# Z-yq/TensorflowASR

Measured on AMD Instinct MI355X. Metric: audio-frames/sec/GPU + RTF, ConformerCTC(S) 10s utts, 1/2/4/8 MI355X, higher is better.
Workload: dtype f32

## Files before the change

### tensorflowasr_amd/csrc/attention_split.hip

```cpp
#include <cstdlib>

#include "common.h"
#include "env.h"
#include "launch.h"
#include "mfma_ops.h"

MI355_SCALAR_F32_BEGIN

namespace {

#ifndef MI355ASR_ATTN_DIAG
#define MI355ASR_ATTN_DIAG 0
#endif
constexpr int ADG = MI355ASR_ATTN_DIAG;
constexpr int HS = 36;
constexpr int TPK = 256;
constexpr int NKT = TPK / 16;
constexpr int NST = TPK / 32;
constexpr int OT = 3;
constexpr int AW = 16;
constexpr int ATH = AW * 64;

template <int TM>
__global__ __launch_bounds__(ATH) void attention_split_kernel(AttnArgs a) {
  static_assert(TM == 3 || ADG == 0, "the timing variants are those of the three-term kernel");
  __shared__ __attribute__((aligned(16))) u32x4_t Kf[TM][NKT][64];
  __shared__ __attribute__((aligned(16))) float Kt[NKT][64];
  __shared__ __attribute__((aligned(16))) u32x4_t Vf[TM][NST][OT][64];
  const float sq = TM == 2 ? a.h2_sq : 1.f, sk = TM == 2 ? a.h2_sk : 1.f, sv = TM == 2 ? a.h2_sv : 1.f;
  constexpr float SP = TM == 2 ? 16384.f : 1.f;

  const int tid = threadIdx.x, lane = tid & 63, wv = tid >> 6;
  const int g = lane >> 4, g4 = g * 4, c = lane & 15;
  const int TS = a.Tk, TQ = a.Tq;
  const int h = blockIdx.y, b = blockIdx.z;
  const int T = a.k_len ? min(a.k_len[b], TS) : TS;
  const int ld = a.ldk, D = a.D;
  const size_t khead = a.head_major ? ((size_t)b * a.H + h) * TS * HS : (size_t)b * TS * ld + h * HS;
  const float* __restrict__ kbase = a.k + khead;
  const float* __restrict__ vbase = a.v + khead;

  const int qt = blockIdx.x * AW + wv;
  const int tq = qt * 16 + c;
  const float* qrow = a.head_major ? a.q + (((size_t)b * a.H + h) * TQ + min(tq, TQ - 1)) * HS
                                   : a.q + ((size_t)b * TQ + min(tq, TQ - 1)) * a.ldq + h * HS;
  constexpr float LOG2E = 1.4426950408889634f;
  const f32x4 qlo = ldg4(qrow + 8 * g), qhi = ldg4(qrow + 8 * g + 4);
  const float qtl = qrow[32 + g] * (LOG2E * sq);

  const int skey = 16 * wv + c;
  const float* krow = kbase + (size_t)min(skey, T - 1) * ld;
  f32x4 klo = ldg4(krow + 8 * g), khi = ldg4(krow + 8 * g + 4);
  float ktl = krow[32 + g];
  constexpr int NVE = NST * OT * 64, NVT = (NVE + ATH - 1) / ATH;
  float ve[NVT][8];
#pragma unroll
  for (int it = 0; it < NVT; ++it) {
    const int en = tid + it * ATH;
    const int s = en / (OT * 64), rem = en - s * (OT * 64), ot = rem >> 6, l = rem & 63, kg = l >> 4, fc = l & 15;
    const int f = 16 * ot + fc;
#pragma unroll
    for (int j = 0; j < 8; ++j) {
      const int key = 32 * s + 16 * (j >> 2) + 4 * kg + (j & 3);
      ve[it][j] = (!(ADG & 16) && en < NVE && f < HS && key < T) ? vbase[(size_t)key * ld + f] : 0.f;
    }
  }
  if (skey >= T) { klo = splat4(0.f); khi = splat4(0.f); ktl = 0.f; }
  {
    const Split8x3 kf = split_tm<TM>(klo * splat4(sk), khi * splat4(sk));
    Kf[0][wv][lane] = kf.t[0];
    Kf[1][wv][lane] = kf.t[1];
    if constexpr (TM == 3) Kf[2][wv][lane] = kf.t[2];
    Kt[wv][lane] = ktl * sk;
  }
  __syncthreads();
  const bool active = qt * 16 < TQ;
  const int nkt = (T + 15) / 16;
  const Split8x3 qf = split_tm<TM>(qlo * splat4(LOG2E * sq), qhi * splat4(LOG2E * sq));
  const f32x4 inv_qk = splat4(1.0f / (sq * sk));

  f32x4 sc[NKT];
  auto qk_tile = [&](int kt) {
    const u32x4_t kf[3] = {Kf[0][kt][lane], Kf[1][kt][lane], Kf[TM - 1][kt][lane]};
    const float kl = Kt[kt][lane];
    if constexpr (ADG & 1) { sc[kt] = splat4(kl) + __builtin_bit_cast(f32x4, kf[0]); return; }
    f32x4 acc = mma_tm<TM>(kf, qf, splat4(0.f));
    sc[kt] = mfma4(kl, qtl, acc);
    if constexpr (TM == 2) sc[kt] = sc[kt] * inv_qk;
  };
  const bool full = (nkt == NKT);
  if (active) {
    if (full) {
#pragma unroll
      for (int kt = 0; kt < NKT; ++kt) qk_tile(kt);
    } else {
#pragma unroll
      for (int kt = 0; kt < NKT; ++kt) {
        if (kt < nkt) qk_tile(kt); else sc[kt] = splat4(-INFINITY);
      }
    }
  }

#pragma unroll
  for (int it = 0; it < NVT; ++it) {
    const int en = tid + it * ATH;
    if (en < NVE && !(ADG & 8)) {
      const f32x4 lo = {ve[it][0], ve[it][1], ve[it][2], ve[it][3]}, hi = {ve[it][4], ve[it][5], ve[it][6], ve[it][7]};
      const Split8x3 vf = split_tm<TM>(lo * splat4(sv), hi * splat4(sv));
      u32x4_t* dst = &Vf[0][0][0][0] + en;
      dst[0] = vf.t[0];
      dst[NVE] = vf.t[1];
      if constexpr (TM == 3) dst[2 * NVE] = vf.t[2];
    }
  }
  if (!active) { __syncthreads(); return; }

  float mx = -INFINITY;
#pragma unroll
  for (int kt = 0; kt < NKT; ++kt) {
    if (kt < nkt && 16 * kt + 16 > T) {
      const int kb = 16 * kt + g4;
      sc[kt].x = (kb + 0 < T) ? sc[kt].x : -INFINITY;
      sc[kt].y = (kb + 1 < T) ? sc[kt].y : -INFINITY;
      sc[kt].z = (kb + 2 < T) ? sc[kt].z : -INFINITY;
      sc[kt].w = (kb + 3 < T) ? sc[kt].w : -INFINITY;
    }
    mx = fmaxf(mx, fmaxf(fmaxf(sc[kt].x, sc[kt].y), fmaxf(sc[kt].z, sc[kt].w)));
  }
  mx = group_max(mx);
  float psum = 0.f;
#pragma unroll
  for (int kt = 0; kt < NKT; ++kt) {
    if constexpr (!(ADG & 2)) {
      sc[kt].x = __builtin_amdgcn_exp2f(sc[kt].x - mx);
      sc[kt].y = __builtin_amdgcn_exp2f(sc[kt].y - mx);
      sc[kt].z = __builtin_amdgcn_exp2f(sc[kt].z - mx);
      sc[kt].w = __builtin_amdgcn_exp2f(sc[kt].w - mx);
    }
    psum += (sc[kt].x + sc[kt].y) + (sc[kt].z + sc[kt].w);
  }

  __syncthreads();
  f32x4 o[OT];
#pragma unroll
  for (int i = 0; i < OT; ++i) o[i] = splat4(0.f);
  const int nst = (nkt + 1) / 2;
#pragma unroll
  for (int s = 0; s < NST; ++s) {
    if constexpr (ADG & 4) { o[0] += sc[2 * s]; o[1] += sc[2 * s + 1]; }
    else if (s < nst) {
      const Split8x3 pf = split_tm<TM>(sc[2 * s] * splat4(SP), sc[2 * s + 1] * splat4(SP));
#pragma unroll
      for (int i = 0; i < OT; ++i) {
        const u32x4_t vf[3] = {Vf[0][s][i][lane], Vf[1][s][i][lane], Vf[TM - 1][s][i][lane]};
        o[i] = mma_tm<TM>(vf, pf, o[i]);
      }
    }
  }
  const float inv = (1.0f / group_sum(psum)) * (1.0f / (SP * sv));
  if (tq < TQ) {
    float* orow = a.ctx + ((size_t)b * TQ + tq) * D + h * HS;
#pragma unroll
    for (int i = 0; i < OT; ++i) {
      if (16 * i + g4 < HS) stg4(orow + 16 * i + g4, o[i] * splat4(inv));
    }
  }
}


constexpr int LKB = 256;
constexpr int LKT = LKB / 16;
constexpr int LST = LKB / 32;
template <int TM, int LW>
__global__ __launch_bounds__(LW * 64) void attention_split_long_kernel(AttnArgs a) {
  constexpr int LTH = LW * 64;
  constexpr bool LPRE = LW <= 8;
  __shared__ __attribute__((aligned(16))) u32x4_t Kf[TM][LKT][64];
  __shared__ __attribute__((aligned(16))) float Kt[LKT][64];
  __shared__ __attribute__((aligned(16))) u32x4_t Vf[TM][LST][OT][64];
  const float sq = TM == 2 ? a.h2_sq : 1.f, sk = TM == 2 ? a.h2_sk : 1.f, sv = TM == 2 ? a.h2_sv : 1.f;
  constexpr float SP = TM == 2 ? 16384.f : 1.f;
  const int tid = threadIdx.x, lane = tid & 63, wv = tid >> 6;
  const int g = lane >> 4, g4 = g * 4, c = lane & 15;
  const int TS = a.Tk, TQ = a.Tq;
  const int h = blockIdx.y, b = blockIdx.z;
  const int T = a.k_len ? min(a.k_len[b], TS) : TS;
  const int ld = a.ldk, D = a.D;
  const size_t khead = a.head_major ? ((size_t)b * a.H + h) * TS * HS : (size_t)b * TS * ld + h * HS;
  const float* __restrict__ kbase = a.k + khead;
  const float* __restrict__ vbase = a.v + khead;
  const int qt = blockIdx.x * LW + wv;
  const int tq = qt * 16 + c;
  const float* qrow = a.head_major ? a.q + (((size_t)b * a.H + h) * TQ + min(tq, TQ - 1)) * HS
                                   : a.q + ((size_t)b * TQ + min(tq, TQ - 1)) * a.ldq + h * HS;
  constexpr float LOG2E = 1.4426950408889634f;
  const f32x4 qlo = ldg4(qrow + 8 * g), qhi = ldg4(qrow + 8 * g + 4);
  const float qtl = qrow[32 + g] * (LOG2E * sq);
  const Split8x3 qf = split_tm<TM>(qlo * splat4(LOG2E * sq), qhi * splat4(LOG2E * sq));
  const f32x4 inv_qk = splat4(1.0f / (sq * sk));
  const bool active = qt * 16 < TQ;

  constexpr int NKE = LKT * 64, NKR = (NKE + LTH - 1) / LTH;
  constexpr int NVE = LST * OT * 64, NVR = (NVE + LTH - 1) / LTH;
  f32x4 klo[NKR], khi[NKR];
  float ktl[NKR];
  float ve[NVR][8];
  const unsigned uld = (unsigned)ld;
  auto fetch = [&](int kb0) {
#pragma unroll
    for (int it = 0; it < NKR; ++it) {
      const int en = tid + it * LTH, kt = en >> 6, l = en & 63, kg = l >> 4, kc = l & 15;
      const int skey = kb0 + 16 * kt + kc;
      const unsigned ko = (unsigned)min(skey, T - 1) * uld + 8u * kg;
      const bool ok = en < NKE && skey < T;
      klo[it] = ok ? *reinterpret_cast<const f32x4*>(kbase + ko) : splat4(0.f);
      khi[it] = ok ? *reinterpret_cast<const f32x4*>(kbase + ko + 4u) : splat4(0.f);
      ktl[it] = ok ? kbase[(unsigned)min(skey, T - 1) * uld + 32u + kg] : 0.f;
    }
#pragma unroll
    for (int it = 0; it < NVR; ++it) {
      const int en = tid + it * LTH;
      const int s = en / (OT * 64), rem = en - s * (OT * 64), ot = rem >> 6, l = rem & 63, kg = l >> 4, fc = l & 15;
      const int f = 16 * ot + fc;
      const int key0 = kb0 + 32 * s + 4 * kg;
      const unsigned vo = (unsigned)key0 * uld + (unsigned)f;
#pragma unroll
      for (int j = 0; j < 8; ++j) {
        const int dk = 16 * (j >> 2) + (j & 3);
        ve[it][j] = (en < NVE && f < HS && key0 + dk < T) ? vbase[vo + (unsigned)dk * uld] : 0.f;
      }
    }
  };
  auto stage = [&]() {
#pragma unroll
    for (int it = 0; it < NKR; ++it) {
      const int en = tid + it * LTH;
      if (en < NKE) {
        const Split8x3 kf = split_tm<TM>(klo[it] * splat4(sk), khi[it] * splat4(sk));
        (&Kf[0][0][0])[en] = kf.t[0];
        (&Kf[1][0][0])[en] = kf.t[1];
        if constexpr (TM == 3) (&Kf[2][0][0])[en] = kf.t[2];
        (&Kt[0][0])[en] = ktl[it] * sk;
      }
    }
#pragma unroll
    for (int it = 0; it < NVR; ++it) {
      const int en = tid + it * LTH;
      if (en < NVE) {
        const f32x4 lo = {ve[it][0], ve[it][1], ve[it][2], ve[it][3]}, hi = {ve[it][4], ve[it][5], ve[it][6], ve[it][7]};
        const Split8x3 vf = split_tm<TM>(lo * splat4(sv), hi * splat4(sv));
        u32x4_t* dst = &Vf[0][0][0][0] + en;
        dst[0] = vf.t[0];
        dst[NVE] = vf.t[1];
        if constexpr (TM == 3) dst[2 * NVE] = vf.t[2];
      }
    }
  };

  float m = -INFINITY, psum = 0.f;
  f32x4 o[OT];
#pragma unroll
  for (int i = 0; i < OT; ++i) o[i] = splat4(0.f);
  if constexpr (LPRE) fetch(0);
#pragma unroll 1
  for (int kb0 = 0; kb0 < T; kb0 += LKB) {
    if constexpr (!LPRE) fetch(kb0);
    stage();
// ... 119 lines not shown
```

### tensorflowasr_amd/csrc/subconv.hip

```cpp
#include <cstdio>
#include <cstdlib>

#include "common.h"
#include "env.h"
#include "launch.h"
#include "wstream.h"
#include "mfma_ops.h"

MI355_SCALAR_F32_BEGIN

namespace {

constexpr int D = 144;
constexpr int KB = D / 16;
constexpr int NB = KB;

struct SubCtx {
  float win[7][7];
  unsigned valid;
  int g4;
  const float *p_w1, *p_b1;
};

struct SubState {
  f32x4 xf;
  f32x4 tw[2][2];
};

DEV f32x4 rd_tap(const float* w1c, int tp) {
  int off = tp * D;
  asm volatile("" : "+v"(off));
  return *reinterpret_cast<const f32x4*>(w1c + off);
}
DEV void tap(f32x4& v, const SubCtx& cx, int q, int tp, const f32x4 w) {
  const int kt = q / 3, kf = q % 3, i = tp / 3, j = tp % 3;
  float m = cx.win[2 * kt + i][2 * kf + j];
  asm volatile("" : "+v"(m));
  v.x = __builtin_fmaf(m, w.x, v.x); v.y = __builtin_fmaf(m, w.y, v.y);
  v.z = __builtin_fmaf(m, w.z, v.z); v.w = __builtin_fmaf(m, w.w, v.w);
}
DEV f32x4 finish(f32x4 v, const SubCtx& cx, int q) {
  const bool ok = (cx.valid >> q) & 1u;
  v.x = ok ? fmaxf(v.x, 0.f) : 0.f; v.y = ok ? fmaxf(v.y, 0.f) : 0.f;
  v.z = ok ? fmaxf(v.z, 0.f) : 0.f; v.w = ok ? fmaxf(v.w, 0.f) : 0.f;
  return v;
}

template <int CUR0>
DEV void channel_block(f32x4 (&acc)[NB], WStream<NB>& ws, SubState& st, unsigned l16, const SubCtx& cx, int cb,
                       const f32x4* __restrict__ w2) {
  const int cbn = min(cb + 1, KB - 1);
  const float* w1c = cx.p_w1 + 16 * cb + cx.g4;
  const float* w1n = cx.p_w1 + 16 * cbn + cx.g4;
  const f32x4 b1v = lds4(cx.p_b1, cb, cx.g4), b1n = lds4(cx.p_b1, cbn, cx.g4);
  static_for<0, 9>([&](auto Q) {
    constexpr int q = decltype(Q)::value;
    constexpr int qn = (q + 1) % 9;
    const int sidx = cb * 9 + q;
    const f32x4* p1 = w2 + (size_t)min(sidx + 1, 9 * KB - 1) * (KB * 64);
    const f32x4* p2 = w2 + (size_t)min(sidx + 2, 9 * KB - 1) * (KB * 64);
    f32x4 xn = (q < 8) ? b1v : b1n;
    batch_step<(CUR0 + q) & 1>(acc, st.xf, ws, l16, p1, p2, [&](auto GI) {
      constexpr int gi = decltype(GI)::value;
      constexpr int h = CUR0 + q * 5 + gi;
      tap(xn, cx, qn, 2 * gi, st.tw[h & 1][0]);
      if constexpr (gi < 4) tap(xn, cx, qn, 2 * gi + 1, st.tw[h & 1][1]);
      if constexpr (gi == 4) xn = finish(xn, cx, qn);
      constexpr int gn = (gi + 1) % 5;
      const float* wsrc = (q < 7 || (q == 7 && gi < 4)) ? w1c : w1n;
      st.tw[(h + 1) & 1][0] = rd_tap(wsrc, 2 * gn);
      if constexpr (gn < 4) st.tw[(h + 1) & 1][1] = rd_tap(wsrc, 2 * gn + 1);
    });
    st.xf = xn;
  });
}

__global__ __launch_bounds__(BLOCK_THREADS, 2) void subconv144_kernel(SubConvArgs a) {
  __shared__ __attribute__((aligned(16))) float p_w1[9 * D], p_b1[D], p_b2[D];
  const int lane = threadIdx.x & 63;
  const int g4 = (lane >> 4) * 4, c = lane & 15;
  const int wid = blockIdx.x * WAVES_PER_BLOCK + (threadIdx.x >> 6);
  const int P = a.B * a.T2 * a.F2;

  SubCtx cx;
  cx.g4 = g4; cx.p_w1 = p_w1; cx.p_b1 = p_b1;
  const int pos = wid * 16 + c;
  {
    const int p = min(pos, P - 1);
    const int b = p / (a.T2 * a.F2);
    const int r = p % (a.T2 * a.F2);
    const int t2 = r / a.F2, f2 = r % a.F2;
    int F = a.F, T1 = a.T1, pt1 = a.pt1, pt2 = a.pt2;
    if (a.wav_len) {
      int t2_;
      F = (a.wav_len[b] + a.hop - 1) / a.hop;
      ragged_same_pad(F, 3, a.st1, &T1, &pt1);
      ragged_same_pad(T1, 3, 2, &t2_, &pt2);
    }
    const int tm0 = 4 * t2 - 2 * pt2 - pt1;
    const int fm0 = 4 * f2 - 2 * a.pf2 - a.pf1;
    const float* __restrict__ mb = a.mel + (size_t)b * a.F * a.NM;
#pragma unroll
    for (int i = 0; i < 7; ++i) {
      const int tm = tm0 + i;
#pragma unroll
      for (int j = 0; j < 7; ++j) {
        const int fm = fm0 + j;
        cx.win[i][j] = (tm >= 0 && tm < F && fm >= 0 && fm < a.NM) ? mb[(size_t)tm * a.NM + fm] : 0.f;
      }
    }
    cx.valid = 0;
#pragma unroll
    for (int kt = 0; kt < 3; ++kt)
#pragma unroll
      for (int kf = 0; kf < 3; ++kf) {
        const int t1 = 2 * t2 + kt - pt2, f1 = 2 * f2 + kf - a.pf2;
        const unsigned ok = (unsigned)((t1 >= 0) & (t1 < T1) & (f1 >= 0) & (f1 < a.F1));
        cx.valid |= ok << (kt * 3 + kf);
      }
  }
  const f32x4* w2 = reinterpret_cast<const f32x4*>(a.w2p);
  WStream<NB> ws;
  ws.lane16 = (unsigned)lane * 16u;
  stream_begin(ws, w2, w2 + (size_t)KB * 64);
  stash(p_w1, a.w1, 9 * D); stash(p_b1, a.b1, D); stash(p_b2, a.b2, D);
  __syncthreads();
  if ((size_t)wid * 16 >= (size_t)P) return;

  f32x4 acc[NB];
#pragma unroll
  for (int n = 0; n < NB; ++n) acc[n] = lds4(p_b2, n, g4);
  SubState st;
  {
    const float* w1c = p_w1 + g4;
    f32x4 v = lds4(p_b1, 0, g4);
#pragma unroll
    for (int tp = 0; tp < 9; ++tp) tap(v, cx, 0, tp, rd_tap(w1c, tp));
    st.xf = finish(v, cx, 0);
    st.tw[0][0] = rd_tap(w1c, 0);
    st.tw[0][1] = rd_tap(w1c, 1);
  }
#pragma unroll 1
  for (int cb = 0; cb + 1 < KB; cb += 2) {
    const unsigned l16 = fresh_lane16(ws.lane16);
    channel_block<0>(acc, ws, st, l16, cx, cb, w2);
    channel_block<1>(acc, ws, st, l16, cx, cb + 1, w2);
  }
  {
    const unsigned l16 = fresh_lane16(ws.lane16);
    channel_block<0>(acc, ws, st, l16, cx, KB - 1, w2);
  }
  if (pos < P) {
    float* orow = a.out + (size_t)pos * D;
#pragma unroll
    for (int n = 0; n < NB; ++n) {
      f32x4 v = acc[n];
      v.x = fmaxf(v.x, 0.f); v.y = fmaxf(v.y, 0.f); v.z = fmaxf(v.z, 0.f); v.w = fmaxf(v.w, 0.f);
      stg4(orow + 16 * n + g4, v);
    }
  }
}


constexpr int SCW = 8, SCT = SCW * 64, SRT = 2, SPOSG = SCW * 16 * SRT;
constexpr int NPAIR = 4;
constexpr int ninth_steps(int kb) { return (kb + 1) / 2; }
constexpr int MELP = 8192;

#ifndef MI355ASR_SUBCONV_C1I
#define MI355ASR_SUBCONV_C1I 1
#endif
#ifndef MI355ASR_SUBCONV_RING
#define MI355ASR_SUBCONV_RING 4
#endif
constexpr int SRING = MI355ASR_SUBCONV_RING;
static_assert(SRING >= 2 && (SRING & (SRING - 1)) == 0, "ring slots: a power of two");
DEV void wait_vmcnt(int n) {
  switch (n) {
    case 0: __builtin_amdgcn_s_waitcnt(0x0f70); break;
    case 2: __builtin_amdgcn_s_waitcnt(0x0f72); break;
    case 3: __builtin_amdgcn_s_waitcnt(0x0f73); break;
    case 4: __builtin_amdgcn_s_waitcnt(0x0f74); break;
    case 6: __builtin_amdgcn_s_waitcnt(0x0f76); break;
    case 8: __builtin_amdgcn_s_waitcnt(0x0f78); break;
    case 9: __builtin_amdgcn_s_waitcnt(0x0f79); break;
    case 12: __builtin_amdgcn_s_waitcnt(0x0f7c); break;
    default: __builtin_amdgcn_s_waitcnt(0x0f70); break;
  }
}

#ifndef MI355ASR_CONV1_V2
#define MI355ASR_CONV1_V2 1
#endif
#define MI355ASR_CONV1_PK MI355ASR_CONV1_V2

template <int RTN, bool PK_ = true>
struct SplitLane {
  static constexpr bool PK = PK_;
  int mb[RTN];
  unsigned valid[RTN];
};

struct PatchGeom { int row, seg; };
#if MI355ASR_CONV1_V2
struct Win9 { float m[3][3]; };
template <int Q, int DIAG = 0, class SL>
DEV Win9 conv1_window(const float* melp, PatchGeom RS, const SL& sl, int rt) {
  constexpr int kt = Q / 3, kf = Q % 3;
  int off = sl.mb[rt];
  asm volatile("" : "+v"(off));
  const float* mp = melp + off + (2 * kt) * RS.row;
  Win9 w;
#pragma unroll
  for (int i = 0; i < 3; ++i) {
    const float* rp = mp + i * RS.row;
    if constexpr (DIAG == 5) {
#pragma unroll
      for (int j = 0; j < 3; ++j) w.m[i][j] = __builtin_bit_cast(float, off + i * RS.row + 2 * kf + j);
    } else if constexpr (kf == 1) {
      const f32x2 a = *reinterpret_cast<const f32x2*>(rp + 2);
      w.m[i][0] = a.x; w.m[i][1] = a.y; w.m[i][2] = rp[4];
    } else {
      const f32x4 a = *reinterpret_cast<const f32x4*>(rp + 2 * kf);
      w.m[i][0] = a.x; w.m[i][1] = a.y; w.m[i][2] = a.z;
    }
  }
  return w;
}
template <int Q, class SL>
DEV f32x4 conv1_eval(const Win9& win, const SL& sl, int rt, const f32x4 (&w1r)[9], f32x4 b1v) {
  f32x2 lo2 = {b1v.x, b1v.y}, hi2 = {b1v.z, b1v.w};
#pragma unroll
  for (int i = 0; i < 3; ++i)
#pragma unroll
    for (int j = 0; j < 3; ++j) {
      const f32x4 w = w1r[i * 3 + j];
      const float m = win.m[i][j];
      if constexpr (SL::PK) {
        const f32x2 mm = {m, m};
        lo2 = __builtin_elementwise_fma(mm, f32x2{w.x, w.y}, lo2);
        hi2 = __builtin_elementwise_fma(mm, f32x2{w.z, w.w}, hi2);
      } else {
        lo2.x = __builtin_fmaf(m, w.x, lo2.x); lo2.y = __builtin_fmaf(m, w.y, lo2.y);
        hi2.x = __builtin_fmaf(m, w.z, hi2.x); hi2.y = __builtin_fmaf(m, w.w, hi2.y);
      }
    }
  const bool ok = (sl.valid[rt] >> Q) & 1u;
  const float lim = ok ? __builtin_inff() : 0.f;
  return f32x4{__builtin_amdgcn_fmed3f(lo2.x, 0.f, lim), __builtin_amdgcn_fmed3f(lo2.y, 0.f, lim),
               __builtin_amdgcn_fmed3f(hi2.x, 0.f, lim), __builtin_amdgcn_fmed3f(hi2.y, 0.f, lim)};
}
template <int Q, int DIAG = 0, class SL>
DEV f32x4 conv1_at(const float* melp, PatchGeom RS, const SL& sl, int rt, const f32x4 (&w1r)[9], f32x4 b1v) {
  return conv1_eval<Q>(conv1_window<Q, DIAG>(melp, RS, sl, rt), sl, rt, w1r, b1v);
}
#else
template <int Q, int DIAG = 0, class SL>
DEV f32x4 conv1_at(const float* melp, PatchGeom RS, const SL& sl, int rt, const f32x4 (&w1r)[9], f32x4 b1v) {
  constexpr int kt = Q / 3, kf = Q % 3;
  f32x4 v = b1v;
  int off = sl.mb[rt];
  asm volatile("" : "+v"(off));
  const float* mp = melp + off + (2 * kt) * RS.row;
#pragma unroll
  for (int i = 0; i < 3; ++i)
#pragma unroll
    for (int j = 0; j < 3; ++j) {
      const int mc = 2 * kf + j, col = (mc & 3) * RS.seg + (mc >> 2);
      const float m = DIAG == 5 ? __builtin_bit_cast(float, off + i * RS.row + col) : mp[i * RS.row + col];
      const f32x4 w = w1r[i * 3 + j];
      v.x = __builtin_fmaf(m, w.x, v.x); v.y = __builtin_fmaf(m, w.y, v.y);
      v.z = __builtin_fmaf(m, w.z, v.z); v.w = __builtin_fmaf(m, w.w, v.w);
    }
  const bool ok = (sl.valid[rt] >> Q) & 1u;
  v.x = ok ? fmaxf(v.x, 0.f) : 0.f; v.y = ok ? fmaxf(v.y, 0.f) : 0.f;
  v.z = ok ? fmaxf(v.z, 0.f) : 0.f; v.w = ok ? fmaxf(v.w, 0.f) : 0.f;
  return v;
}
#endif

template <int PAIR, int DIAG = 0, int TM = 3, int RTN, class SL>
DEV void frags_for(Split8x3 (&xf)[RTN], const float* melp, PatchGeom RS, const SL& sl, const f32x4 (&w1r)[9], f32x4 b1v) {
#pragma unroll
  for (int rt = 0; rt < RTN; ++rt) {
    f32x4 lo, hi;
#if MI355ASR_CONV1_V2
    if constexpr (SL::PK) {
      const Win9 wlo = conv1_window<2 * PAIR, DIAG>(melp, RS, sl, rt), whi = conv1_window<2 * PAIR + 1, DIAG>(melp, RS, sl, rt);
      lo = conv1_eval<2 * PAIR>(wlo, sl, rt, w1r, b1v);
      hi = conv1_eval<2 * PAIR + 1>(whi, sl, rt, w1r, b1v);
    } else
#endif
    {
      lo = conv1_at<2 * PAIR, DIAG>(melp, RS, sl, rt, w1r, b1v);
      hi = conv1_at<2 * PAIR + 1, DIAG>(melp, RS, sl, rt, w1r, b1v);
    }
    if constexpr (DIAG == 6) {
      const u32x4_t l = __builtin_bit_cast(u32x4_t, lo), h = __builtin_bit_cast(u32x4_t, hi);
      xf[rt].t[0] = l; xf[rt].t[1] = h; xf[rt].t[2] = l ^ h;
    } else {
      xf[rt] = split_tm<TM>(lo, hi);
    }
  }
}

template <int DIAG, int TM, class LT, int RTN, class SL>
DEV void frags_ninth(Split8x3 (&xf)[RTN], const float* melp, PatchGeom RS, const SL& sl, f32x4 (&w1r)[9], const float* p_b1,
                     int g4, int cbA, int KBn, LT&& load_taps) {
  f32x4 lo[RTN], hi[RTN];
  load_taps(cbA);
#pragma unroll
  for (int rt = 0; rt < RTN; ++rt) lo[rt] = conv1_at<8, DIAG>(melp, RS, sl, rt, w1r, lds4(p_b1, cbA, g4));
  if (cbA + 1 < KBn) {
    load_taps(cbA + 1);
#pragma unroll
    for (int rt = 0; rt < RTN; ++rt) hi[rt] = conv1_at<8, DIAG>(melp, RS, sl, rt, w1r, lds4(p_b1, cbA + 1, g4));
  } else {
#pragma unroll
    for (int rt = 0; rt < RTN; ++rt) hi[rt] = splat4(0.f);
  }
#pragma unroll
  for (int rt = 0; rt < RTN; ++rt) xf[rt] = split_tm<TM>(lo[rt], hi[rt]);
}

constexpr int C1_ROWB = 192;
constexpr int C1_ZERO_ROWS = 8;
template <int RTN>
struct C1Lane {
  static constexpr bool PK = true;
// ... 69 lines not shown
    load_taps(cbA + 1);
    const u32x4_t ah = c1_place<2>(tp.ph, tp.qh), al = c1_place<2>(tp.pl, tp.ql);
    const f32x4 c0v = lds4(p_b1, cbA + 1, g4);
#pragma unroll
    for (int rt = 0; rt < RTN; ++rt) hi[rt] = mma32h(al, wh[rt], c0v);
#pragma unroll
    for (int rt = 0; rt < RTN; ++rt) hi[rt] = mma32h(ah, wlo[rt], hi[rt]);
#pragma unroll
    for (int rt = 0; rt < RTN; ++rt) hi[rt] = mma32h(ah, wh[rt], hi[rt]);
#pragma unroll
    for (int rt = 0; rt < RTN; ++rt) hi[rt] = c1_finish<8>(hi[rt], sl, rt, kmul);
  } else {
#pragma unroll
    for (int rt = 0; rt < RTN; ++rt) hi[rt] = splat4(0.f);
  }
#pragma unroll
  for (int rt = 0; rt < RTN; ++rt) xf[rt] = split_tm<2>(c1_finish<8>(lo[rt], sl, rt, kmul), hi[rt]);
}

template <int DIAG, int DM, int NBW, int TM = 3, int RTN = SRT, bool C1M = false>
__global__ __launch_bounds__(SCT, 2) void subconv_split_ring_kernel(SubConvArgs a, PatchGeom RS, int rows) {
  static_assert(DIAG == 0 || RTN == SRT, "the timing variants run two row tiles per wave");
  static_assert(!C1M || (TM == 2 && (DM == 144 || DM == 256)), "conv1 on the matrix pipe: the two-term kernels of dmodel 144 / 256");
  constexpr int KB = DM / 16, NB = NBW, NI = ninth_steps(KB), NK32 = KB * NPAIR + NI, SLABF = NBW * TM * 64, D = DM;
  const int c0 = blockIdx.z * NBW;
  __shared__ __attribute__((aligned(16))) u32x4_t wl[SRING][SLABF];
  __shared__ __attribute__((aligned(16))) float melp[MELP];
  __shared__ __attribute__((aligned(16))) float p_w1[9 * D], p_b1[D], p_b2[D];
  const int lane = threadIdx.x & 63, wave = threadIdx.x >> 6;
  const int g4 = (lane >> 4) * 4, c = lane & 15;
  const int b = blockIdx.y, r0 = blockIdx.x * (SCW * 16 * RTN), PU = a.T2 * a.F2;
  int F = a.F, T1 = a.T1, pt1 = a.pt1, pt2 = a.pt2;
  if (a.wav_len) {
    int t2_;
    F = (a.wav_len[b] + a.hop - 1) / a.hop;
    ragged_same_pad(F, 3, a.st1, &T1, &pt1);
    ragged_same_pad(T1, 3, 2, &t2_, &pt2);
  }
  const u32x4_t* __restrict__ wg = reinterpret_cast<const u32x4_t*>(TM == 2 ? a.w2h : a.w2s) + (size_t)blockIdx.z * NK32 * SLABF;
  float s1 = TM == 2 ? a.h_scale : 1.f;
  if (TM == 2 && a.h_melmax) {
    const float bound = fmaf(a.h_l1, __uint_as_float(a.h_melmax[b]), a.h_bmax);
    const int e = (int)((__float_as_uint(bound) >> 23) & 255u);
    s1 = __uint_as_float((unsigned)(127 + min(60, max(-60, 141 - e))) << 23);
  }
  const float s2 = TM == 2 ? s1 * a.h_wscale : 1.f;
  float sm = 1.f, kmul = 1.f;
  if constexpr (C1M) {
    sm = a.c1_mscale;
    if (a.h_melmax) {
      const int e = (int)((a.h_melmax[b] >> 23) & 255u);
      sm = __uint_as_float((unsigned)(127 + min(60, max(-60, 141 - e))) << 23);
    }
    kmul = s1 / (sm * a.c1_wscale);
  }
  constexpr int NQ = (SLABF + SCT - 1) / SCT;
  u32x4_t nw[NQ];
#pragma unroll
  for (int q = 0; q < NQ; ++q) {
    const int idx = threadIdx.x + SCT * q;
    nw[q] = u32x4_t{0u, 0u, 0u, 0u};
    if (idx < SLABF) nw[q] = wg[idx];
  }
  const int t2a = r0 / a.F2;
  const int tm_base = 4 * t2a - 2 * pt2 - pt1, fm_base = -2 * a.pf2 - a.pf1;
  const float* __restrict__ mbp = a.mel + (size_t)b * a.F * a.NM;
  const int RSL = 4 * RS.seg;
  const unsigned plane = (unsigned)rows * C1_ROWB;
  const unsigned melp_addr = (unsigned)(size_t)(__attribute__((address_space(3))) void*)melp;
  if constexpr (C1M) {
    unsigned* mph = reinterpret_cast<unsigned*>(melp);
    constexpr int RD = C1_ROWB / 4;
    for (int i = threadIdx.x; i < rows * RD; i += SCT) {
      const int rr = i / RD, jp = i - rr * RD;
      const int tm = tm_base + rr, fm = fm_base + 2 * jp;
      const bool okr = tm >= 0 && tm < F;
      const float v0 = (okr && fm >= 0 && fm < a.NM) ? mbp[(size_t)tm * a.NM + fm] * sm : 0.f;
      const float v1 = (okr && fm + 1 >= 0 && fm + 1 < a.NM) ? mbp[(size_t)tm * a.NM + fm + 1] * sm : 0.f;
      const unsigned h = split_hi_f16(v0, v1);
      mph[i] = h;
      mph[rows * RD + i] = split_lo_f16(h, v0, v1);
    }
    for (int i = threadIdx.x; i < C1_ZERO_ROWS * RD; i += SCT) mph[2 * rows * RD + i] = 0u;
  } else {
  for (int i = threadIdx.x; i < rows * RSL; i += SCT) {
    const int rr = i / RSL, jj = i - rr * RSL;
    const int tm = tm_base + rr, fm = fm_base + jj;
    melp[MI355ASR_CONV1_V2 ? rr * RS.row + jj : rr * RS.row + (jj & 3) * RS.seg + (jj >> 2)] =
        (tm >= 0 && tm < F && fm >= 0 && fm < a.NM) ? mbp[(size_t)tm * a.NM + fm] : 0.f;
  }
  }
  {
    const float ws1 = C1M ? a.c1_wscale : s1, bs1 = C1M ? sm * a.c1_wscale : s1;
    for (int i = threadIdx.x; i < 9 * D; i += SCT) p_w1[i] = a.w1[i] * ws1;
    for (int i = threadIdx.x; i < D; i += SCT) { p_b1[i] = a.b1[i] * bs1; p_b2[i] = a.b2[i] * s2; }
  }
  std::conditional_t<C1M, C1Lane<RTN>, SplitLane<RTN, DM == 144>> sl;
#pragma unroll
  for (int rt = 0; rt < RTN; ++rt) {
    const int r = min(r0 + 16 * RTN * wave + 16 * rt + c, PU - 1);
    const int t2 = r / a.F2, f2 = r - t2 * a.F2;
    if constexpr (C1M) {
      const int g = lane >> 4;
      const unsigned win = melp_addr + (unsigned)(4 * (t2 - t2a) + g) * C1_ROWB + 8u * (unsigned)f2;
      const unsigned zero = melp_addr + 2u * plane;
      sl.bh[rt] = g < 3 ? win : zero;
      sl.bl[rt] = g < 3 ? win + plane : zero;
    } else {
      sl.mb[rt] = 4 * (t2 - t2a) * RS.row + (MI355ASR_CONV1_V2 ? 4 * f2 : f2);
    }
    unsigned vm = 0;
#pragma unroll
    for (int kt = 0; kt < 3; ++kt)
#pragma unroll
      for (int kf = 0; kf < 3; ++kf) {
        const int t1 = 2 * t2 + kt - pt2, f1 = 2 * f2 + kf - a.pf2;
        vm |= (unsigned)((t1 >= 0) & (t1 < T1) & (f1 >= 0) & (f1 < a.F1)) << (kt * 3 + kf);
      }
    sl.valid[rt] = vm;
  }
#pragma unroll
  for (int q = 0; q < NQ; ++q) {
    const int idx = threadIdx.x + SCT * q;
    if (idx < SLABF) wl[0][idx] = nw[q];
  }
  __syncthreads();

  f32x4 acc[RTN][NB];
#pragma unroll
  for (int n = 0; n < NB; ++n) {
    const f32x4 bv = lds4(p_b2, c0 + n, g4);
#pragma unroll
    for (int rt = 0; rt < RTN; ++rt) acc[rt][n] = bv;
  }
  f32x4 w1r[C1M ? 1 : 9];
  C1Taps c1t{0u, 0u, 0u, 0u};
  auto load_taps = [&](int cb) {
    if constexpr (C1M) {
      const int g = lane >> 4;
      const float* wp = p_w1 + 3 * min(g, 2) * D + 16 * cb + c;
      const float w0 = g < 3 ? wp[0] : 0.f, w1 = g < 3 ? wp[D] : 0.f, w2 = g < 3 ? wp[2 * D] : 0.f;
      c1t.ph = split_hi_f16(w0, w1);
      c1t.qh = split_hi_f16(w2, 0.f);
      c1t.pl = split_lo_f16(c1t.ph, w0, w1);
      c1t.ql = split_lo_f16(c1t.qh, w2, 0.f);
    } else {
#pragma unroll
      for (int tp = 0; tp < 9; ++tp) w1r[tp] = *reinterpret_cast<const f32x4*>(p_w1 + tp * D + 16 * cb + g4);
    }
  };
  auto sl_bh = [&](int rt) { if constexpr (C1M) return sl.bh[rt]; else return 0u; };
  auto sl_bl = [&](int rt) { if constexpr (C1M) return sl.bl[rt]; else return 0u; };
  constexpr bool C1I = C1M && MI355ASR_SUBCONV_C1I;
  Split8x3 xbuf[C1I ? 2 : 1][RTN];
  Split8x3 (&xa)[RTN] = xbuf[0];
  auto frags_pair = [&](auto PI, int cb, auto DST) {
    constexpr int pair = decltype(PI)::value;
    Split8x3 (&dst)[RTN] = xbuf[C1I ? decltype(DST)::value : 0];
    if constexpr (C1M) frags_for_mm<pair>(dst, sl, c1t, lds4(p_b1, cb, g4), kmul);
    else frags_for<pair, DIAG, TM>(dst, melp, RS, sl, w1r, lds4(p_b1, cb, g4));
  };
  auto frags_9th = [&](int cbA, auto DST) {
    Split8x3 (&dst)[RTN] = xbuf[C1I ? decltype(DST)::value : 0];
    if constexpr (C1M) frags_ninth_mm(dst, sl, c1t, p_b1, g4, cbA, KB, kmul, load_taps);
    else frags_ninth<DIAG, TM>(dst, melp, RS, sl, w1r, p_b1, g4, cbA, KB, load_taps);
  };
  using B0 = std::integral_constant<int, 0>;
  u32x4_t c1w[4];
  f32x4 c1v[2];
  auto c1_piece = [&](auto PI, auto GI, int cb, auto DST) {
    constexpr int pair = decltype(PI)::value, gi = decltype(GI)::value, QA = 2 * pair, QB = 2 * pair + 1;
    Split8x3 (&dst)[RTN] = xbuf[C1I ? decltype(DST)::value : 0];
    auto reads = [&](int rt) {
      c1w[0] = c1_read<QA / 3>(sl_bh(rt)); c1w[1] = c1_read<QA / 3>(sl_bl(rt));
      c1w[2] = c1_read<QB / 3>(sl_bh(rt)); c1w[3] = c1_read<QB / 3>(sl_bl(rt));
    };
    auto conv = [&]() {
      asm volatile("" : "+v"(c1w[0]), "+v"(c1w[1]), "+v"(c1w[2]), "+v"(c1w[3]));
      const f32x4 c0v = lds4(p_b1, cb, g4);
      const u32x4_t ahA = c1_place<QA % 3>(c1t.ph, c1t.qh), alA = c1_place<QA % 3>(c1t.pl, c1t.ql);
      const u32x4_t ahB = c1_place<QB % 3>(c1t.ph, c1t.qh), alB = c1_place<QB % 3>(c1t.pl, c1t.ql);
      c1v[0] = mma32h(alA, c1w[0], c0v); c1v[1] = mma32h(alB, c1w[2], c0v);
      c1v[0] = mma32h(ahA, c1w[1], c1v[0]); c1v[1] = mma32h(ahB, c1w[3], c1v[1]);
      c1v[0] = mma32h(ahA, c1w[0], c1v[0]); c1v[1] = mma32h(ahB, c1w[2], c1v[1]);
    };
    auto finish = [&](int rt) { dst[rt] = split_tm<2>(c1_finish<QA>(c1v[0], sl, rt, kmul), c1_finish<QB>(c1v[1], sl, rt, kmul)); };
    if constexpr (gi == 0) reads(0);
    else if constexpr (gi == 1) conv();
    else if constexpr (gi == 2) { finish(0); if constexpr (RTN > 1) reads(1); }
    else if constexpr (gi == 3) { if constexpr (RTN > 1) conv(); }
    else if constexpr (gi == 4) { if constexpr (RTN > 1) finish(1); }
  };
  if constexpr (DIAG == 1) {
#pragma unroll
    for (int rt = 0; rt < RTN; ++rt)
#pragma unroll
      for (int t = 0; t < 3; ++t) xa[rt].t[t] = u32x4_t{0x3f803f80u, 0x3f803f80u, 0x3f803f80u, 0x3f803f80u};
  }
  const int wv = __builtin_amdgcn_readfirstlane(wave);
  const bool late = wv >= SCW / 2;
  int my_pieces = 0;
#pragma unroll
  for (int q = 0; q < NQ; ++q) my_pieces += (SCT * q + 64 * wv < SLABF) ? 1 : 0;
  auto issue_slab = [&](int t) {
    if (t < NK32 && DIAG != 3) {
      const u32x4_t* src = wg + (size_t)t * SLABF;
#pragma unroll
      for (int q = 0; q < NQ; ++q) {
        const int w0 = SCT * q + 64 * wv;
        if (w0 < SLABF) dma16(src + w0 + lane, &wl[t & (SRING - 1)][w0]);
      }
    }
  };
  for (int t = 1; t <= SRING - 2; ++t) issue_slab(t);
  auto run = [&](auto LATE_T) {
  constexpr bool LATE = decltype(LATE_T)::value || C1I;
  if constexpr (LATE) {
    load_taps(0);
    frags_pair(B0{}, 0, B0{});
  }
  auto step_body = [&](int s, auto&& frags_this, auto&& frags_next, auto PAR_T) {
      const int cur = s & (SRING - 1);
      Split8x3 (&xin)[RTN] = xbuf[(C1M && MI355ASR_SUBCONV_C1I) ? decltype(PAR_T)::value : 0];
      auto slab_dma = [&]() { issue_slab(s + SRING - 1); };
      auto mfma_cur = [&](auto&& between) {
        constexpr int G = NB % 2 == 0 ? 2 : 1, NG = NB / G;
        const unsigned base = (unsigned)(size_t)(__attribute__((address_space(3))) void*)(&wl[cur][lane]);
        u32x4_t wa[G][3], wb[G][3];
        auto fetch = [&](u32x4_t (&w)[G][3], auto GI) {
          constexpr int gi = decltype(GI)::value;
          static_for<0, G>([&](auto HI) {
            constexpr int h = decltype(HI)::value;
            if constexpr (DIAG == 9 && gi > 0) { w[h][0] = wa[0][0]; w[h][1] = wa[0][1]; if constexpr (TM == 3) w[h][2] = wa[0][2]; return; }
            w[h][0] = lds_read16<((gi * G + h) * TM + 0) * 1024>(base);
            w[h][1] = lds_read16<((gi * G + h) * TM + 1) * 1024>(base);
            if constexpr (TM == 3) w[h][2] = lds_read16<((gi * G + h) * TM + 2) * 1024>(base);
          });
        };
        auto wait = [&](u32x4_t (&w)[G][3], auto N_T) {
          constexpr int N = decltype(N_T)::value;
          if constexpr (TM == 2 && G == 1)
            asm volatile("s_waitcnt lgkmcnt(%2)" : "+v"(w[0][0]), "+v"(w[0][1]) : "n"(N));
          else if constexpr (TM == 2)
            asm volatile("s_waitcnt lgkmcnt(%4)" : "+v"(w[0][0]), "+v"(w[0][1]), "+v"(w[1][0]), "+v"(w[1][1]) : "n"(N));
          else if constexpr (G == 1)
            asm volatile("s_waitcnt lgkmcnt(%3)" : "+v"(w[0][0]), "+v"(w[0][1]), "+v"(w[0][2]) : "n"(N));
          else
            asm volatile("s_waitcnt lgkmcnt(%6)" : "+v"(w[0][0]), "+v"(w[0][1]), "+v"(w[0][2]), "+v"(w[1][0]), "+v"(w[1][1]),
                         "+v"(w[1][2]) : "n"(N));
        };
        auto mma = [&](const u32x4_t (&w)[G][3], auto GI) {
          constexpr int gi = decltype(GI)::value;
#pragma unroll
          for (int ord = DIAG == 7 ? 1 : TM - 1; ord >= 0; --ord)
#pragma unroll
            for (int p = 0; p <= ord; ++p)
#pragma unroll
              for (int h = 0; h < G; ++h)
#pragma unroll
                for (int rt = 0; rt < RTN; ++rt) {
                  if constexpr (DIAG == 8)
                    acc[rt][gi * G + h] += __builtin_bit_cast(f32x4, w[h][ord - p] ^ xin[rt].t[p]);
                  else
                    acc[rt][gi * G + h] = mma32_tm<TM>(w[h][ord - p], xin[rt].t[p], acc[rt][gi * G + h]);
                }
        };
        fetch(wa, std::integral_constant<int, 0>{});
        static_for<0, NG>([&](auto GI) {
          constexpr int gi = decltype(GI)::value;
          if constexpr (gi % 2 == 0) {
            if constexpr (gi + 1 < NG) { fetch(wb, std::integral_constant<int, gi + 1>{}); wait(wa, std::integral_constant<int, TM * G>{}); }
            else wait(wa, std::integral_constant<int, 0>{});
            mma(wa, GI);
            between(GI);
          } else {
            if constexpr (gi + 1 < NG) { fetch(wa, std::integral_constant<int, gi + 1>{}); wait(wb, std::integral_constant<int, TM * G>{}); }
            else wait(wb, std::integral_constant<int, 0>{});
            mma(wb, GI);
            between(GI);
          }
        });
      };
      auto nothing = [](auto) {};
      if constexpr (DIAG == 1) {
        slab_dma();
        mfma_cur(nothing);
      } else if constexpr (C1M && MI355ASR_SUBCONV_C1I) {
        mfma_cur([&](auto GI) {
          if constexpr (decltype(GI)::value == 0) {
            __builtin_amdgcn_sched_barrier(0);
            slab_dma();
            __builtin_amdgcn_sched_barrier(0);
          }
          frags_this(GI);
        });
        constexpr int NGR = NB / (NB % 2 == 0 ? 2 : 1);
        if constexpr (NGR < 5) static_for<NGR, 5>([&](auto GI) { frags_this(GI); });
        __builtin_amdgcn_sched_barrier(0);
        frags_next();
      } else if constexpr (LATE) {
        mfma_cur([&](auto GI) {
          if constexpr (decltype(GI)::value == 0) {
            __builtin_amdgcn_sched_barrier(0);
            slab_dma();
            __builtin_amdgcn_sched_barrier(0);
          }
        });
        __builtin_amdgcn_sched_barrier(0);
        frags_next();
      } else {
        frags_this();
        __builtin_amdgcn_sched_barrier(0);
        slab_dma();
        __builtin_amdgcn_sched_barrier(0);
        mfma_cur(nothing);
      }
      {
        const int behind = min(SRING - 2, NK32 - 2 - s);
        wait_vmcnt(DIAG == 3 ? 0 : max(behind, 0) * my_pieces);
      }
      if constexpr (DIAG != 4) {
        __builtin_amdgcn_sched_barrier(0);
        __builtin_amdgcn_s_waitcnt(0xc07f);
        __builtin_amdgcn_s_barrier();
        __builtin_amdgcn_sched_barrier(0);
      }
  };
#pragma unroll 1
  for (int cb = 0; cb < KB; ++cb) {
    static_for<0, NPAIR>([&](auto PI) {
      constexpr int pair = decltype(PI)::value;
      using PAR = std::integral_constant<int, pair & 1>;
      using NXT = std::integral_constant<int, (pair & 1) ^ 1>;
      if constexpr (C1I) {
        step_body(cb * NPAIR + pair,
                  [&](auto GI) {
                    if constexpr (pair + 1 < NPAIR) c1_piece(std::integral_constant<int, pair + 1>{}, GI, cb, NXT{});
                    else if (cb + 1 < KB) {
                      if constexpr (decltype(GI)::value == 0) load_taps(cb + 1);
                      c1_piece(B0{}, GI, cb + 1, NXT{});
                    }
                  },
                  [&]() { if constexpr (pair + 1 == NPAIR) { if (cb + 1 == KB) frags_9th(0, NXT{}); } },
                  PAR{});
      } else {
      step_body(cb * NPAIR + pair,
                [&]() {
                  if constexpr (pair == 0) load_taps(cb);
                  frags_pair(PI, cb, B0{});
                },
                [&]() {
                  if constexpr (pair + 1 < NPAIR) {
                    frags_pair(std::integral_constant<int, pair + 1>{}, cb, B0{});
                  } else if (cb + 1 < KB) {
                    load_taps(cb + 1);
                    frags_pair(B0{}, cb + 1, B0{});
                  } else {
                    frags_9th(0, B0{});
                  }
                }, B0{});
      }
    });
  }
  if constexpr (C1I) {
    static_assert((KB * NPAIR) % 2 == 0, "the first ninth-tap step reads operand buffer 0");
    static_for<0, NI>([&](auto II) {
      constexpr int i = decltype(II)::value;
      step_body(KB * NPAIR + i, [](auto) {}, [&]() { if constexpr (i + 1 < NI) frags_9th(2 * i + 2, std::integral_constant<int, (i & 1) ^ 1>{}); },
                std::integral_constant<int, i & 1>{});
    });
  } else {
#pragma unroll 1
  for (int i = 0; i < NI; ++i) {
    step_body(KB * NPAIR + i,
              [&]() { frags_9th(2 * i, B0{}); },
              [&]() { if (i + 1 < NI) frags_9th(2 * i + 2, B0{}); }, B0{});
  }
  }
  };
  if (late || C1I) run(std::integral_constant<bool, true>{});
  else run(std::integral_constant<bool, false>{});
  const float inv2 = 1.0f / s2;
#pragma unroll
  for (int rt = 0; rt < RTN; ++rt) {
    const int r = r0 + 16 * RTN * wave + 16 * rt + c;
    if (r < PU) {
      float* orow = a.out + ((size_t)b * PU + r) * D;
#pragma unroll
      for (int n = 0; n < NB; ++n) {
        f32x4 v = acc[rt][n];
        v.x = fmaxf(v.x, 0.f); v.y = fmaxf(v.y, 0.f); v.z = fmaxf(v.z, 0.f); v.w = fmaxf(v.w, 0.f);
        if constexpr (TM == 2) v = v * splat4(inv2);
        stg4(orow + 16 * (c0 + n) + g4, v);
      }
    }
  }
}

}

int launch_subconv144(const SubConvArgs& a, hipStream_t s) {
  const int P = a.B * a.T2 * a.F2;
  const int tiles = (P + 15) / 16;
  hipLaunchKernelGGL(subconv144_kernel, dim3((tiles + 3) / 4), dim3(BLOCK_THREADS), 0, s, a);
  return 0;
}

template <int DIAG>
static int launch_split_d(int d, const dim3& g144, const SubConvArgs& a, PatchGeom RS, int rows, hipStream_t s, int rtn = SRT) {
  const dim3 g128(g144.x, g144.y, d / 128);
  note_scheme(SCHEME_BF16X3);
  if constexpr (DIAG == 0) {
    static const bool c1m_env = mi355_env("MI355ASR_SUBCONV_C1M", 1) != 0;
    const bool c1m = c1m_env && a.w2h && (d == 144 || d == 256) && a.c1_wscale > 0.f && (a.c1_mscale > 0.f || a.h_melmax) && 4 * a.F2 + 4 <= C1_ROWB / 2 &&
                     (size_t)(2 * rows + C1_ZERO_ROWS) * C1_ROWB <= sizeof(float) * MELP;
    if (c1m) {
      note_scheme(SCHEME_F16X2);
      if (d == 256) {
        if (rtn == 1) hipLaunchKernelGGL((subconv_split_ring_kernel<0, 256, 8, 2, 1, true>), g128, dim3(SCT), 0, s, a, RS, rows);
        else hipLaunchKernelGGL((subconv_split_ring_kernel<0, 256, 8, 2, SRT, true>), g128, dim3(SCT), 0, s, a, RS, rows);
      } else if (rtn == 1) hipLaunchKernelGGL((subconv_split_ring_kernel<0, 144, 9, 2, 1, true>), g144, dim3(SCT), 0, s, a, RS, rows);
      else hipLaunchKernelGGL((subconv_split_ring_kernel<0, 144, 9, 2, SRT, true>), g144, dim3(SCT), 0, s, a, RS, rows);
      return 0;
    }
    if (a.w2h && rtn == 1) {
      note_scheme(SCHEME_F16X2);
      switch (d) {
        case 144: hipLaunchKernelGGL((subconv_split_ring_kernel<0, 144, 9, 2, 1>), g144, dim3(SCT), 0, s, a, RS, rows); return 0;
        case 256: hipLaunchKernelGGL((subconv_split_ring_kernel<0, 256, 8, 2, 1>), g128, dim3(SCT), 0, s, a, RS, rows); return 0;
        case 512: hipLaunchKernelGGL((subconv_split_ring_kernel<0, 512, 8, 2, 1>), g128, dim3(SCT), 0, s, a, RS, rows); return 0;
        default: return -1;
      }
    }
    if (a.w2h) {
      note_scheme(SCHEME_F16X2);
      switch (d) {
        case 144: hipLaunchKernelGGL((subconv_split_ring_kernel<0, 144, 9, 2>), g144, dim3(SCT), 0, s, a, RS, rows); return 0;
        case 256: hipLaunchKernelGGL((subconv_split_ring_kernel<0, 256, 8, 2>), g128, dim3(SCT), 0, s, a, RS, rows); return 0;
        case 512: hipLaunchKernelGGL((subconv_split_ring_kernel<0, 512, 8, 2>), g128, dim3(SCT), 0, s, a, RS, rows); return 0;
        default: return -1;
      }
    }
  }
  if constexpr (DIAG != 0) {
    if (a.w2h && d == 144) {
      note_scheme(SCHEME_F16X2);
      hipLaunchKernelGGL((subconv_split_ring_kernel<DIAG, 144, 9, 2>), g144, dim3(SCT), 0, s, a, RS, rows);
      return 0;
    }
  }
  switch (d) {
    case 144: hipLaunchKernelGGL((subconv_split_ring_kernel<DIAG, 144, 9>), g144, dim3(SCT), 0, s, a, RS, rows); return 0;
    case 256: hipLaunchKernelGGL((subconv_split_ring_kernel<DIAG, 256, 8>), g128, dim3(SCT), 0, s, a, RS, rows); return 0;
    case 512: hipLaunchKernelGGL((subconv_split_ring_kernel<DIAG, 512, 8>), g128, dim3(SCT), 0, s, a, RS, rows); return 0;
    default: return -1;
  }
}

int launch_subconv_split(int d, const SubConvArgs& a, hipStream_t s) {
  const int PU = a.T2 * a.F2;
  PatchGeom RS;
  RS.seg = a.F2 + 1;
  RS.row = 4 * RS.seg;
#if MI355ASR_CONV1_V2
  while (RS.row % 4 != 0) ++RS.row;
  if (a.F2 % 4 == 0)
    while (RS.row % 8 != a.F2 % 8) RS.row += 4;
#else
  while (RS.row % 8 != 5) ++RS.row;
#endif
  static const int rt_env = (int)mi355_env("MI355ASR_SUBCONV_RT", 0);
  const long wg1 = (long)((PU + SPOSG / 2 - 1) / (SPOSG / 2)) * a.B * (d == 144 ? 1 : d / 128);
  const int rtn = (a.w2h && (rt_env == 1 || (rt_env == 0 && wg1 <= 256))) ? 1 : SRT;
  const int posg = SCW * 16 * rtn;
  const int span = (posg - 1 + a.F2 - 1) / a.F2;
  const int rows = 4 * span + 7;
  if ((!a.w2s && !a.w2h) || a.st1 != 2 || rows * RS.row > MELP || PU <= 0) return -1;
  const dim3 grid((PU + posg - 1) / posg, a.B);
#ifdef MI355ASR_DIAG_KERNELS
// ... 24 lines not shown
```

Before: 35.22 million.

## Stagger wave barriers in subconv ring pipeline; add optional attention V-staging stagger

In the subsampling conv kernel, the late half of the waves now reaches the per-step barrier partway through the MFMA group loop, while the early waves hit it after the step. To keep the slot being overwritten safe, the DMA prefetch distance is shortened by one ring slot. The aim is to desynchronise the two wave halves so LDS reads, MFMA and DMA issue spread out rather than all waves stalling at the barrier together. In the attention kernel, an optional (default-off) mode has half the waves stage V before QK, plus optional setprio knobs; this trades prefetch depth for less barrier convoying.

```diff
diff --git a/tensorflowasr_amd/csrc/attention_split.hip b/tensorflowasr_amd/csrc/attention_split.hip
--- a/tensorflowasr_amd/csrc/attention_split.hip
+++ b/tensorflowasr_amd/csrc/attention_split.hip
@@ -13,6 +13,12 @@
 #define MI355ASR_ATTN_DIAG 0
 #endif
 constexpr int ADG = MI355ASR_ATTN_DIAG;
+#ifndef MI355ASR_ATTN_STAGGER
+#define MI355ASR_ATTN_STAGGER 0
+#endif
+#ifndef MI355ASR_ATTN_STAGGER_PRIO
+#define MI355ASR_ATTN_STAGGER_PRIO 0
+#endif
 constexpr int HS = 36;
 constexpr int TPK = 256;
 constexpr int NKT = TPK / 16;
@@ -88,6 +94,26 @@
     sc[kt] = mfma4(kl, qtl, acc);
     if constexpr (TM == 2) sc[kt] = sc[kt] * inv_qk;
   };
+  auto stage_v = [&]() {
+#pragma unroll
+    for (int it = 0; it < NVT; ++it) {
+      const int en = tid + it * ATH;
+      if (en < NVE && !(ADG & 8)) {
+        const f32x4 lo = {ve[it][0], ve[it][1], ve[it][2], ve[it][3]}, hi = {ve[it][4], ve[it][5], ve[it][6], ve[it][7]};
+        const Split8x3 vf = split_tm<TM>(lo * splat4(sv), hi * splat4(sv));
+        u32x4_t* dst = &Vf[0][0][0][0] + en;
+        dst[0] = vf.t[0];
+        dst[NVE] = vf.t[1];
+        if constexpr (TM == 3) dst[2 * NVE] = vf.t[2];
+      }
+    }
+  };
+  constexpr bool STG = MI355ASR_ATTN_STAGGER && TM == 2;
+  const bool vfirst = STG && __builtin_amdgcn_readfirstlane(wv) >= AW / 2;
+  if (vfirst) {
+    if constexpr (STG && MI355ASR_ATTN_STAGGER_PRIO) __builtin_amdgcn_s_setprio(1);
+    stage_v();
+  }
   const bool full = (nkt == NKT);
   if (active) {
     if (full) {
@@ -101,18 +127,7 @@
     }
   }
 
-#pragma unroll
-  for (int it = 0; it < NVT; ++it) {
-    const int en = tid + it * ATH;
-    if (en < NVE && !(ADG & 8)) {
-      const f32x4 lo = {ve[it][0], ve[it][1], ve[it][2], ve[it][3]}, hi = {ve[it][4], ve[it][5], ve[it][6], ve[it][7]};
-      const Split8x3 vf = split_tm<TM>(lo * splat4(sv), hi * splat4(sv));
-      u32x4_t* dst = &Vf[0][0][0][0] + en;
-      dst[0] = vf.t[0];
-      dst[NVE] = vf.t[1];
-      if constexpr (TM == 3) dst[2 * NVE] = vf.t[2];
-    }
-  }
+  if (!vfirst) stage_v();
   if (!active) { __syncthreads(); return; }
 
   float mx = -INFINITY;
diff --git a/tensorflowasr_amd/csrc/subconv.hip b/tensorflowasr_amd/csrc/subconv.hip
--- a/tensorflowasr_amd/csrc/subconv.hip
+++ b/tensorflowasr_amd/csrc/subconv.hip
@@ -175,6 +175,16 @@
 #endif
 constexpr int SRING = MI355ASR_SUBCONV_RING;
 static_assert(SRING >= 2 && (SRING & (SRING - 1)) == 0, "ring slots: a power of two");
+#ifndef MI355ASR_SUBCONV_STAGGER
+#define MI355ASR_SUBCONV_STAGGER 1
+#endif
+#ifndef MI355ASR_SUBCONV_STAGGER_GROUP
+#define MI355ASR_SUBCONV_STAGGER_GROUP 7
+#endif
+static_assert(MI355ASR_SUBCONV_STAGGER_GROUP >= 0 && MI355ASR_SUBCONV_STAGGER_GROUP < 8, "a fragment group in front of the step's last");
+#ifndef MI355ASR_SUBCONV_STAGGER_PRIO
+#define MI355ASR_SUBCONV_STAGGER_PRIO 0
+#endif
 DEV void wait_vmcnt(int n) {
   switch (n) {
     case 0: __builtin_amdgcn_s_waitcnt(0x0f70); break;
@@ -550,6 +560,8 @@
   auto sl_bh = [&](int rt) { if constexpr (C1M) return sl.bh[rt]; else return 0u; };
   auto sl_bl = [&](int rt) { if constexpr (C1M) return sl.bl[rt]; else return 0u; };
   constexpr bool C1I = C1M && MI355ASR_SUBCONV_C1I;
+  constexpr bool STAG = MI355ASR_SUBCONV_STAGGER && C1I && DIAG == 0 && DM == 144 && RTN == SRT && SRING >= 4;
+  constexpr int SDIST = SRING - 1 - (STAG ? 1 : 0);
   Split8x3 xbuf[C1I ? 2 : 1][RTN];
   Split8x3 (&xa)[RTN] = xbuf[0];
   auto frags_pair = [&](auto PI, int cb, auto DST) {
@@ -610,7 +622,8 @@
       }
     }
   };
-  for (int t = 1; t <= SRING - 2; ++t) issue_slab(t);
+  for (int t = 1; t <= SDIST - 1; ++t) issue_slab(t);
+  if constexpr (STAG && MI355ASR_SUBCONV_STAGGER_PRIO) { if (late) __builtin_amdgcn_s_setprio(1); }
   auto run = [&](auto LATE_T) {
   constexpr bool LATE = decltype(LATE_T)::value || C1I;
   if constexpr (LATE) {
@@ -620,7 +633,17 @@
   auto step_body = [&](int s, auto&& frags_this, auto&& frags_next, auto PAR_T) {
       const int cur = s & (SRING - 1);
       Split8x3 (&xin)[RTN] = xbuf[(C1M && MI355ASR_SUBCONV_C1I) ? decltype(PAR_T)::value : 0];
-      auto slab_dma = [&]() { issue_slab(s + SRING - 1); };
+      auto slab_dma = [&]() { issue_slab(s + SDIST); };
+      auto step_sync = [&]() {
+        const int behind = min(SDIST - 1, NK32 - 2 - s);
+        wait_vmcnt(DIAG == 3 ? 0 : max(behind, 0) * my_pieces);
+        if constexpr (DIAG != 4) {
+          __builtin_amdgcn_sched_barrier(0);
+          __builtin_amdgcn_s_waitcnt(0xc07f);
+          __builtin_amdgcn_s_barrier();
+          __builtin_amdgcn_sched_barrier(0);
+        }
+      };
       auto mfma_cur = [&](auto&& between) {
         constexpr int G = NB % 2 == 0 ? 2 : 1, NG = NB / G;
         const unsigned base = (unsigned)(size_t)(__attribute__((address_space(3))) void*)(&wl[cur][lane]);
@@ -691,6 +714,7 @@
             __builtin_amdgcn_sched_barrier(0);
           }
           frags_this(GI);
+          if constexpr (STAG && decltype(GI)::value == MI355ASR_SUBCONV_STAGGER_GROUP) { if (late) step_sync(); }
         });
         constexpr int NGR = NB / (NB % 2 == 0 ? 2 : 1);
         if constexpr (NGR < 5) static_for<NGR, 5>([&](auto GI) { frags_this(GI); });
@@ -713,16 +737,8 @@
         __builtin_amdgcn_sched_barrier(0);
         mfma_cur(nothing);
       }
-      {
-        const int behind = min(SRING - 2, NK32 - 2 - s);
-        wait_vmcnt(DIAG == 3 ? 0 : max(behind, 0) * my_pieces);
-      }
-      if constexpr (DIAG != 4) {
-        __builtin_amdgcn_sched_barrier(0);
-        __builtin_amdgcn_s_waitcnt(0xc07f);
-        __builtin_amdgcn_s_barrier();
-        __builtin_amdgcn_sched_barrier(0);
-      }
+      if constexpr (STAG) { if (!late) step_sync(); }
+      else step_sync();
   };
 #pragma unroll 1
   for (int cb = 0; cb < KB; ++cb) {
```

Measured after the change: 35.32 million (median of 2 runs). About the same (+0.3%).
